# frank-xwang/InstanceDiffusion

Measured on AMD Instinct MI355X. Metric: images/sec at 512x512, 50 PLMS steps, N=8 instances (Multi-instance Sampler), higher is better.
Workload: dtype bf16; 1 GPU; C3: SD-1.5 InstanceDiffusion UNet (1.228B params, seeded random weights), 64x64 latent (512x512), 50 PLMS steps, CFG 7.5, N=8 boxes, MIS 0.36, alpha [0.8,0,0.2]; images_per_gpu=32, unet_forwards_per_image=406

## Files before the change

### include/idf.h

```cpp
#ifndef IDF_H_
#define IDF_H_

#include <stdint.h>

#ifdef __cplusplus
extern "C" {
#endif

#define IDF_ABI_VERSION 5

enum { IDF_BF16 = 0, IDF_F16 = 1 };
enum { IDF_E_ARG = -1, IDF_E_ALIGN = -2, IDF_E_UNSUPPORTED = -3 };

enum {
  IDF_EPI_BIAS     = 1,
  IDF_EPI_ROWBIAS  = 2,
  IDF_EPI_RES      = 4,
  IDF_EPI_GATE     = 8,
  IDF_EPI_SILU     = 16,
  IDF_EPI_GELU     = 32,
  IDF_EPI_GEGLU    = 64,
  IDF_EPI_OUT_F32  = 128,
  IDF_EPI_OUT_NCHW = 256,
  IDF_EPI_LN_ROW   = 512,
  IDF_EPI_LN_COL   = 1024,
  IDF_EPI_GEGLU_P32 = 2048
};

int idf_abi_version(void);
const char* idf_build_info(void);

enum { IDF_TUNE_GEMM_BIG = 0, IDF_TUNE_ATTN2 = 1, IDF_TUNE_GEMM_RING = 2, IDF_TUNE_BIG_MIN_EFF = 3, IDF_TUNE_ATTN8 = 4, IDF_TUNE_MLP = 5,
       IDF_TUNE_QKV_ROW = 6, IDF_TUNE_GEGLU_ROW = 7 };
int idf_set_tuning(int knob, int value);
enum { IDF_STAT_GEMM_BIG_LAUNCHES = 0, IDF_STAT_ATTN2_LAUNCHES = 1, IDF_STAT_GEMM_RING_LAUNCHES = 2, IDF_STAT_ATTN8_LAUNCHES = 3,
       IDF_STAT_GN_EPI_LAUNCHES = 4 ,
       IDF_STAT_QKV_ROW_LAUNCHES = 6 ,
       IDF_STAT_GEGLU_ROW_LAUNCHES = 7  };
long long idf_get_stat(int stat);

typedef struct {
  const void* A; const void* W; void* out;
  const float* bias; const void* rowbias; const void* res; const float* gate;
  int M, N, K;
  int lda, ldw, ldo, ldr, ld_rowbias;
  int rows_per_batch;
  int batch; long long strideA, strideW, strideO, strideR;
  int epi; int dtype;
  void* ws; long long ws_bytes;
  const float* ln_stats; long long stride_ln_stats;
  const float* ln_c;
  const float* ln_d;
  float* out_stats; float out_stats_eps;
  float ln_eps; float* ln_stats_out;
  void* vt_out; int ld_vt; int vt_col0;
} idf_gemm_args;
int idf_gemm(const idf_gemm_args* a, void* stream);

typedef struct {
  const void* x; int ldx;
  const float* ln_stats;
  const void* w1; int ldw1;
  const float* cd;
  const void* w2p; int ldw2;
  const float* b2;
  const float* gate;
  void* out; int ldo;
  int M, C;
  int dtype;
} idf_mlp_args;
int idf_mlp_geglu(const idf_mlp_args* a, void* stream);

int idf_row_stats(const void* x, int ldx, float* stats, int M, int C, float eps, int dtype, void* stream);

typedef struct {
  const void* x; const void* W; void* out;
  const float* bias; const void* rowbias; const void* res;
  int B, Hin, Win, Cin, Cout;
  int stride;
  int upsample;
  int ldx, ldo, ldr, ld_rowbias;
  int n_valid;
  int epi; int dtype;
  void* ws; long long ws_bytes;
  float* gn_partial;
} idf_conv3x3_args;
int idf_conv3x3(const idf_conv3x3_args* a, void* stream);
int idf_conv3x3_down(const idf_conv3x3_args* a, void* stream);
int idf_conv_up2x_folded(const idf_conv3x3_args* a, void* stream);

int idf_conv_in(const float* x_nchw, const float* w , const float* bias, void* out,
                int B, int Cin, int H, int W, int Cout, int dtype, void* stream);

typedef struct {
// ... 64 lines not shown
```

### instancediffusion_amd/_lib.py

```python
from __future__ import annotations

import ctypes as C
import os

_HERE = os.path.dirname(os.path.abspath(__file__))
LIB_PATH = os.environ.get("IDF_LIB_PATH", os.path.join(_HERE, "libidf_gfx950.so"))

IDF_BF16, IDF_F16 = 0, 1
IDF_STAT_GEMM_BIG_LAUNCHES, IDF_STAT_ATTN2_LAUNCHES, IDF_STAT_GEMM_RING_LAUNCHES, IDF_STAT_ATTN8_LAUNCHES, IDF_STAT_GN_EPI_LAUNCHES = 0, 1, 2, 3, 4
IDF_STAT_QKV_ROW_LAUNCHES, IDF_STAT_GEGLU_ROW_LAUNCHES = 6, 7
IDF_TUNE_GEMM_BIG, IDF_TUNE_ATTN2, IDF_TUNE_GEMM_RING, IDF_TUNE_BIG_MIN_EFF, IDF_TUNE_ATTN8, IDF_TUNE_MLP, IDF_TUNE_QKV_ROW, IDF_TUNE_GEGLU_ROW = 0, 1, 2, 3, 4, 5, 6, 7
EPI_LN_ROW, EPI_LN_COL, EPI_GEGLU_P32 = 512, 1024, 2048
EPI_BIAS, EPI_ROWBIAS, EPI_RES, EPI_GATE, EPI_SILU, EPI_GELU, EPI_GEGLU, EPI_OUT_F32, EPI_OUT_NCHW = \
    1, 2, 4, 8, 16, 32, 64, 128, 256

vp, ll, ci, cf = C.c_void_p, C.c_longlong, C.c_int, C.c_float


class GemmArgs(C.Structure):
    _fields_ = [("A", vp), ("W", vp), ("out", vp), ("bias", vp), ("rowbias", vp), ("res", vp), ("gate", vp),
                ("M", ci), ("N", ci), ("K", ci),
                ("lda", ci), ("ldw", ci), ("ldo", ci), ("ldr", ci), ("ld_rowbias", ci),
                ("rows_per_batch", ci),
                ("batch", ci), ("strideA", ll), ("strideW", ll), ("strideO", ll), ("strideR", ll),
                ("epi", ci), ("dtype", ci), ("ws", vp), ("ws_bytes", ll),
                ("ln_stats", vp), ("stride_ln_stats", ll), ("ln_c", vp), ("ln_d", vp),
                ("out_stats", vp), ("out_stats_eps", cf),
                ("ln_eps", cf), ("ln_stats_out", vp),
                ("vt_out", vp), ("ld_vt", ci), ("vt_col0", ci)]


E_UNSUPPORTED = -3


class ConvArgs(C.Structure):
    _fields_ = [("x", vp), ("W", vp), ("out", vp), ("bias", vp), ("rowbias", vp), ("res", vp),
                ("B", ci), ("Hin", ci), ("Win", ci), ("Cin", ci), ("Cout", ci),
                ("stride", ci), ("upsample", ci),
                ("ldx", ci), ("ldo", ci), ("ldr", ci), ("ld_rowbias", ci),
                ("n_valid", ci), ("epi", ci), ("dtype", ci), ("ws", vp), ("ws_bytes", ll), ("gn_partial", vp)]


class AttnArgs(C.Structure):
    _fields_ = [("q", vp), ("ldq", ci), ("strideQ", ll), ("nq", ci),
                ("k0", vp), ("ldk0", ci), ("strideK0", ll), ("vt0", vp), ("ldv0", ci), ("strideV0", ll), ("n0", ci),
                ("k1", vp), ("ldk1", ci), ("strideK1", ll), ("vt1", vp), ("ldv1", ci), ("strideV1", ll), ("n1", ci),
                ("out", vp), ("ldo", ci), ("strideO", ll),
                ("B", ci), ("H", ci), ("d", ci), ("scale", cf), ("dtype", ci),
                ("qbits", vp), ("strideQb", ll), ("kbits0", vp), ("strideKb0", ll), ("kbits1", vp), ("strideKb1", ll)]


class MlpArgs(C.Structure):
    _fields_ = [("x", vp), ("ldx", ci), ("ln_stats", vp), ("w1", vp), ("ldw1", ci), ("cd", vp), ("w2p", vp), ("ldw2", ci),
                ("b2", vp), ("gate", vp), ("out", vp), ("ldo", ci), ("M", ci), ("C", ci), ("dtype", ci)]


SYMBOLS = {
    "idf_abi_version": (ci, []),
    "idf_build_info": (C.c_char_p, []),
    "idf_set_tuning": (ci, [ci, ci]),
    "idf_get_stat": (ll, [ci]),
    "idf_gemm": (ci, [C.POINTER(GemmArgs), vp]),
    "idf_conv3x3": (ci, [C.POINTER(ConvArgs), vp]),
    "idf_conv3x3_down": (ci, [C.POINTER(ConvArgs), vp]),
    "idf_conv_up2x_folded": (ci, [C.POINTER(ConvArgs), vp]),
    "idf_mlp_geglu": (ci, [C.POINTER(MlpArgs), vp]),
    "idf_conv_in": (ci, [vp, vp, vp, vp, ci, ci, ci, ci, ci, ci, vp]),
    "idf_attention": (ci, [C.POINTER(AttnArgs), vp]),
    "idf_groupnorm_ws_floats": (ll, [ci, ci]),
    "idf_groupnorm": (ci, [vp, vp, vp, vp, vp, ci, ci, ci, cf, ci, ci, vp]),
    "idf_groupnorm_stats": (ci, [vp, vp, ci, ci, ci, ci, ci, vp]),
    "idf_groupnorm_apply": (ci, [vp, vp, vp, vp, vp, ci, ci, ci, ci, cf, ci, ci, vp]),
    "idf_layernorm": (ci, [vp, ci, vp, ci, vp, vp, ci, ci, cf, ci, vp]),
    "idf_row_stats": (ci, [vp, ci, vp, ci, ci, cf, ci, vp]),
    "idf_layernorm_patch2": (ci, [vp, vp, ci, vp, vp, ci, ci, ci, ci, cf, ci, vp]),
    "idf_seg_in_conv": (ci, [vp, vp, vp, vp, ci, ci, ci, ci, ci, vp]),
    "idf_dwconv7x7": (ci, [vp, vp, vp, vp, ci, ci, ci, ci, ci, vp]),
    "idf_scaleu_concat": (ci, [vp, vp, vp, vp, vp, vp, ci, ci, ci, ci, ci, ci, vp]),
    "idf_timestep_embedding": (ci, [vp, vp, ci, ci, ci, vp]),
    "idf_unifusion_embed": (ci, [vp, vp, vp, vp, vp, vp, vp, vp, ci, ci, ci, ci, vp]),
    "idf_cfg_combine": (ci, [vp, vp, cf, vp, ll, vp]),
    "idf_plms_update": (ci, [vp, vp, vp, vp, vp, vp, ci, cf, cf, cf, vp, ll, vp]),
    "idf_mis_merge": (ci, [vp, vp, vp, ci, ci, ci, ci, ci, ci, vp]),
    "idf_cast_f32_to_16": (ci, [vp, vp, ll, ci, vp]),
    "idf_softmax_rows": (ci, [vp, vp, ll, ci, ll, ll, cf, ci, vp]),
    "idf_pointwise_nchw": (ci, [vp, vp, vp, vp, ci, ci, ci, ll, cf, vp]),
    "idf_vae_posterior": (ci, [vp, vp, vp, vp, cf, vp, vp, ci, ci, ci, ll, vp]),
}

# ... 34 lines not shown
```

### instancediffusion_amd/csrc/gemm_conv.hip

```cpp
#include "gemm_core.h"
#include "attn_core.h"
#include <cstdlib>

using namespace idfcore;

namespace {

#ifndef IDF_GEMM_BIG_DEFAULT
#define IDF_GEMM_BIG_DEFAULT 1
#endif
constexpr int LSTR = 72;

template <int DT, int BM, int BN, int WM, int WN, int KLOOP_LDS_BYTES>
__device__ __forceinline__ void tile_epilogue(const CoreParams& p, f32x16 (&acc)[WN / 32][WM / 32], unsigned short* smem,
                                              int m0, int n0, int bz, int wm, int wn, int lane, int wave) {
  constexpr int TM = WM / 32, TN = WN / 32;
  const int l31 = lane & 31, hi = lane >> 5;
  constexpr int CSTR = WN + 4;
  static_assert(4 * WM * CSTR * 4 <= KLOOP_LDS_BYTES, "C staging must fit in the allocated LDS");
  __syncthreads();
  float* Cl = reinterpret_cast<float*>(smem) + wave * (WM * CSTR);
#pragma unroll
  for (int a = 0; a < TN; ++a)
#pragma unroll
// ... 812 lines not shown
    g_ring_tiles = value;
    return prev;
  }
  if (knob == IDF_TUNE_BIG_MIN_EFF) {
    if (value < 1 || value > 100) return IDF_E_ARG;
    return idf_big_min_eff_pct(value);
  }
  if (knob == IDF_TUNE_ATTN2) {
    if (value < 0 || value > 6) return IDF_E_ARG;
    return idf_attn2_set_mode(value);
  }
  if (knob == IDF_TUNE_ATTN8) {
    if (value < 0 || value > 6) return IDF_E_ARG;
    return idf_attn8_set_mode(value);
  }
  if (knob == IDF_TUNE_GEGLU_ROW) {
    if (value < 0 || value > 1) return IDF_E_ARG;
    return idf_gegluw_set_mode(value);
  }
  if (knob == IDF_TUNE_QKV_ROW) {
    if (value < 0 || value > 1) return IDF_E_ARG;
    return idf_qkvw_set_mode(value);
  }
  if (knob == IDF_TUNE_MLP) {
    if (value < 0 || value > 1) return IDF_E_ARG;
    return idf_mlp_set_mode(value);
  }
  return IDF_E_ARG;
}

extern "C" long long idf_get_stat(int stat) {
  if (stat == IDF_STAT_GEMM_BIG_LAUNCHES) return idf_stat_big_launches.load();
  if (stat == IDF_STAT_ATTN2_LAUNCHES) return idf_stat_attn2_launches.load();
  if (stat == IDF_STAT_GEMM_RING_LAUNCHES) return idf_stat_ring_launches.load();
  if (stat == IDF_STAT_ATTN8_LAUNCHES) return idf_stat_attn8_launches.load();
  if (stat == IDF_STAT_GN_EPI_LAUNCHES) return idf_stat_gn_epi_launches.load();
  if (stat == IDF_STAT_QKV_ROW_LAUNCHES) return idf_stat_qkvw_launches.load();
  if (stat == IDF_STAT_GEGLU_ROW_LAUNCHES) return idf_stat_gegluw_launches.load();
  return -1;
}

extern "C" int idf_gemm(const idf_gemm_args* a, void* stream) {
  if (!a || !a->A || !a->W || !a->out) return IDF_E_ARG;
  if (a->M <= 0 || a->N <= 0 || a->K <= 0 || (a->K % BK) != 0) return IDF_E_ARG;
  if ((a->lda % 8) || (a->ldw % 8) || !aligned16(a->A) || !aligned16(a->W)) return IDF_E_ALIGN;
  if ((a->epi & IDF_EPI_GATE) && !(a->epi & IDF_EPI_RES)) return IDF_E_ARG;
// ... 153 lines not shown
```

### instancediffusion_amd/csrc/gemm_core.h

```cpp
#pragma once
#include "common.h"
#include <atomic>

namespace idfcore {

struct CoreParams {
  const unsigned short* W; int ldw; long long strideW; int N;
  const unsigned short* A; int lda; long long strideA; int M; int K;
  int Hin, Win, Cin, Ho, Wo, stride, up;
  void* out; int ldo; long long strideO;
  const float* bias; const unsigned short* rowbias; int ld_rowbias; int rows_per_batch;
  const unsigned short* res; int ldr; long long strideR;
  const float* gate; int epi; int n_valid;
  float* ws; size_t ws_bytes; int splitk; int kt_per_slice;
  int full_items; int kt_full; int tail_m0; int tail_rows;
  const float* ln_stats; long long stride_ln_stats; const float* ln_c; const float* ln_d;
  float ln_eps; float* ln_stats_out;
  unsigned short* vt_out; int ld_vt; int vt_col0;
  float* stat_parts; int parts;
  float* gn_partial; int gn_hw;
  int tile_walk; int dephase; int dephase_units; int epi_vmcnt;
  int pad_lo;
  int fold_tiles;
};
// ... 79 lines not shown
    if (full && ((p.ldo & 7) == 0)) {
      *reinterpret_cast<u32x4*>(o) = pack8<DT>(v);
    } else {
#pragma unroll
      for (int e = 0; e < 8; ++e) if (n + e < p.N) o[e] = Elem<DT>::from_f32(v[e]);
    }
  }
}


}

#define IDF_BIG_UNSUPPORTED (-100)
extern std::atomic<long long> idf_stat_big_launches;
int idf_launch_big(const idfcore::CoreParams& p, int dtype, bool conv, bool force, hipStream_t s, int* splitk_out,
                   int* parts_out = nullptr, int* tail_m0_out = nullptr, int* gst_out = nullptr);
int idf_launch_big_fold(const idfcore::CoreParams& p, int dtype, bool force, hipStream_t s);
int idf_launch_qkv320w(const idfcore::CoreParams& p, int dtype, hipStream_t s);
int idf_launch_geglu640w(const idfcore::CoreParams& p, int dtype, hipStream_t s);
int idf_gegluw_set_mode(int v);
int idf_launch_qkv640w(const idfcore::CoreParams& p, int dtype, hipStream_t s);
int idf_qkvw_set_mode(int v);
int idf_mlp_set_mode(int v);
int idf_big_min_eff_pct(int set);
int idf_num_cu();
int idf_stats_finalize(const float* stat_parts, int parts, int cols_per_part, float* out_stats, int M, float eps, hipStream_t s);
```

### instancediffusion_amd/engine.py

```python
from __future__ import annotations

import os
from typing import Dict, List, Optional, Sequence, Tuple

import torch

from .host.attention import SpatialTransformer
from .host.unet import Downsample, ResBlock, UNetModel, Upsample

LN_SELF_MODE = int(os.environ.get("IDF_LN_SELF", "1"))
if LN_SELF_MODE not in (0, 1, 2):
    raise ValueError(f"IDF_LN_SELF={LN_SELF_MODE}: must be 0, 1 or 2")
QKV_ROW = os.environ.get("IDF_QKV_ROW", "1") != "0"
OBJ_TOKENS = 184
MASK_RES = 64


def _round_up(x: int, m: int) -> int:
    return (x + m - 1) // m * m


GEGLU_PERIOD = int(os.environ.get("IDF_GEGLU_PERIOD", "32"))
if GEGLU_PERIOD not in (32, 64):
    raise ValueError(f"IDF_GEGLU_PERIOD={GEGLU_PERIOD}: must be 32 or 64")
MLP_FUSED = os.environ.get("IDF_MLP_FUSED", "1")
if MLP_FUSED not in ("0", "1"):
    raise ValueError(f"IDF_MLP_FUSED={MLP_FUSED}: must be 0 or 1")
MLP_FUSED = MLP_FUSED == "1" and GEGLU_PERIOD == 32
MLP_MIN_M = int(os.environ.get("IDF_MLP_MIN_M", "32768"))
PAIR_HOIST = os.environ.get("IDF_PAIR_HOIST", "1")
if PAIR_HOIST not in ("0", "1"):
    raise ValueError(f"IDF_PAIR_HOIST={PAIR_HOIST}: must be 0 or 1")
PAIR_HOIST = PAIR_HOIST == "1"
GN_EPI = os.environ.get("IDF_GN_EPI", "1")
if GN_EPI not in ("0", "1"):
    raise ValueError(f"IDF_GN_EPI={GN_EPI}: must be 0 or 1")
GN_EPI = GN_EPI == "1"
UP_FOLD = os.environ.get("IDF_UP_FOLD", "1")
if UP_FOLD not in ("0", "1"):
    raise ValueError(f"IDF_UP_FOLD={UP_FOLD}: must be 0 or 1")
UP_FOLD = UP_FOLD == "1"
DEBUG_PAIRED = os.environ.get("IDF_DEBUG_PAIRED", "0") == "1"


def pack_geglu(w: torch.Tensor, b: torch.Tensor, period: int = 64) -> Tuple[torch.Tensor, torch.Tensor]:
    n2, k = w.shape
    n = n2 // 2
    h = period // 2
    assert n % h == 0
    wv, wg = w[:n].reshape(n // h, h, k), w[n:].reshape(n // h, h, k)
    bv, bg = b[:n].reshape(n // h, h), b[n:].reshape(n // h, h)
    return torch.cat([wv, wg], dim=1).reshape(n2, k).contiguous(), torch.cat([bv, bg], dim=1).reshape(n2).contiguous()


def pack_conv3x3(w: torch.Tensor) -> torch.Tensor:
    co, ci = w.shape[0], w.shape[1]
    return w.permute(0, 2, 3, 1).reshape(co, 9 * ci).contiguous()


def pack_conv_up2x(w: torch.Tensor) -> torch.Tensor:
    assert w.dim() == 4 and tuple(w.shape[2:]) == (3, 3) and w.dtype == torch.float32
    co, ci = w.shape[0], w.shape[1]
    rows = ((w[:, :, 0], w[:, :, 1] + w[:, :, 2]), (w[:, :, 0] + w[:, :, 1], w[:, :, 2]))
    out = w.new_empty(4, co, 4 * ci)
    for py in range(2):
        for px in range(2):
            taps = []
            for ty in range(2):
                r = rows[py][ty]
                cols = (r[:, :, 0], r[:, :, 1] + r[:, :, 2]) if px == 0 else (r[:, :, 0] + r[:, :, 1], r[:, :, 2])
                taps += [cols[0], cols[1]]
            out[py * 2 + px] = torch.stack(taps, dim=1).reshape(co, 4 * ci)
    return out


class _Lin:
    __slots__ = ("w", "b")

    def __init__(self, w, b):
        self.w, self.b = w, b


class Cond:

    _next_uid = 0

    def __init__(self, B: int):
        Cond._next_uid += 1
        self.uid = Cond._next_uid
        self.B = B
        self.objs: Optional[torch.Tensor] = None
        self.k_ctx: List[torch.Tensor] = []
        self.vt_ctx: List[torch.Tensor] = []
        self.k_obj: List[torch.Tensor] = []
        self.vt_obj: List[torch.Tensor] = []
        self.n_ctx = 0
# ... 99 lines not shown
    def _pack_ff(self, ff, norm):
        w = ff.net[0].proj.weight.detach().float()
        g, b = norm.weight.detach().float(), norm.bias.detach().float()
        wp, dp = pack_geglu(w * g[None, :], ff.net[0].proj.bias.detach().float() + w @ b, GEGLU_PERIOD)
        w16 = self._w16(wp)
        f = dict(w1=w16, b1=self._f32(dp), c1=w16.float().sum(1).contiguous(), l2=self._lin(ff.net[2]))
        C = w.shape[1]
        if MLP_FUSED and hasattr(self.ops, "mlp_geglu") and self.ops.mlp_supported(128, C):
            f["cd"], f["w2p"] = self.ops.mlp_pack(w16, f["c1"], f["b1"], f["l2"].w)
        return f

    def _attn(self, a, norm, self_attn: bool):
        d = dict(out=self._lin(a.to_out[0]))
        if self_attn:
            w3, c3, d3 = self._fold_ln(torch.cat([a.to_q.weight.detach(), a.to_k.weight.detach(), a.to_v.weight.detach()], 0),
                                       None, norm)
            C2 = 2 * a.to_q.weight.shape[0]
            d["wqkv"], d["cqkv"], d["dqkv"] = w3, c3, d3
            d["wqk"], d["cqk"], d["dqk"] = w3[:C2], c3[:C2], d3[:C2]
            d["wv"], d["cv"], d["dv"] = w3[C2:], c3[C2:], d3[C2:]
        else:
            d["wq"], d["cq"], d["dq"] = self._fold_ln(a.to_q.weight, None, norm)
            d["wk"], d["wv"] = self._w16(a.to_k.weight), self._w16(a.to_v.weight)
        return d

    def _attn_kv_plain(self, a):
        return dict(wk=self._w16(a.to_k.weight), wv=self._w16(a.to_v.weight))

    def _pack_res(self, rb: ResBlock, emb_w: list, emb_b: list, off: list):
        p = dict(kind="res", cin=rb.channels, cout=rb.out_channels,
                 gn1=(self._f32(rb.in_layers[0].weight), self._f32(rb.in_layers[0].bias)),
                 conv1=self._conv(rb.in_layers[2]),
                 gn2=(self._f32(rb.out_layers[0].weight), self._f32(rb.out_layers[0].bias)),
                 conv2=self._conv(rb.out_layers[3]),
                 skip=None if isinstance(rb.skip_connection, torch.nn.Identity) else self._lin(rb.skip_connection),
                 emb_off=off[0])
        emb_w.append(rb.emb_layers[1].weight.detach().float())
        emb_b.append(rb.emb_layers[1].bias.detach().float())
        off[0] += rb.out_channels
        return p

    def _pack_st(self, st: SpatialTransformer, tanh_alphas: list):
        blk = st.transformer_blocks[0]
        fz = blk.fuser
        idx = len(tanh_alphas)
        tanh_alphas.append(torch.stack([torch.tanh(fz.alpha_attn.detach().float()),
# ... 347 lines not shown
        y = ops.gemm(g.view(M, C), p["proj_in"].w, self.buf("st.x", (M, C)), bias=p["proj_in"].b, out_stats=pqkv)
        att = self._self_attn(p["attn1"], y, st, B, N, C)
        ops.gemm(att.view(M, C), p["attn1"]["out"].w, y, bias=p["attn1"]["out"].b, res=y,
                 out_stats=pqkv if fuser_on else pre)
        if dup:
            x, y = self._dup(x, "st.x_in2"), self._dup(y.view(B, N, C), "st.x2").view(2 * M, C)
            if (pqkv if fuser_on else pre) is not None:
                st = self._dup(st.view(B, N, 2), "st.stats2").view(2 * M, 2)
                pre = st if pre is not None else None
                pqkv = st if pqkv is not None else None
                ffs = st if ffs is not None else None
            else:
                st = self.buf("st.stats", (2 * M, 2), torch.float32)
                ffs = st if ffs is not None else None
            B, M = 2 * B, 2 * M
        i = p["idx"]
        if fuser_on:
            vis = cond.vis if (cond.vis and N == MASK_RES * MASK_RES) else None
            att = self._self_attn(p["f_attn"], y, st, B, N, C, kv_extra=(cond.k_obj[i], cond.vt_obj[i]), vis=vis)
            ops.gemm(att.view(M, C), p["f_attn"]["out"].w, y, bias=p["f_attn"]["out"].b, res=y, gate=self.gates[i, 0:1],
                     out_stats=ffs)
            self._ff(p["f_ff"], y, st, M, C, gate=self.gates[i, 1:2], out_stats=pre)
        a2 = p["attn2"]
        q = ops.gemm(y, a2["wq"], self.buf("st.q", (M, C)), bias=a2["dq"],
                     ln_row=(None if own else st, a2["cq"])).view(B, N, C)
        att = self.buf("st.att", (B, N, C))
        ops.attention(q, cond.k_ctx[i], cond.vt_ctx[i], cond.n_ctx, att, self.heads)
        ops.gemm(att.view(M, C), a2["out"].w, y, bias=a2["out"].b, res=y, out_stats=ffs)
        self._ff(p["ff"], y, st, M, C)
        ops.gemm(y, p["proj_out"].w, x.view(M, C), bias=p["proj_out"].b, res=x.view(M, C))
        return x

    def _run_block(self, layers, h, x_nchw, emb_all, cond, fuser_on, out_role, dup_st: bool = False, gnp=None, next_kind=None):
        for j, p in enumerate(layers):
            k = p["kind"]
            nxt = layers[j + 1]["kind"] if j + 1 < len(layers) else next_kind
            norm_next = nxt in ("res", "st")
            if k == "conv_in":
                B, _, H, W = x_nchw.shape
                h = self.ops.conv_in(x_nchw, p["w"], p["b"], self.buf(out_role, (B, H, W, p["w"].shape[0])))
                gnp = None
            elif k == "res":
                h, gnp = self._res(p, h, emb_all, out_role, gnp, want_out=norm_next)
            elif k == "st":
                h = self._st(p, h, cond, fuser_on, dup=dup_st, gnp=gnp)
                gnp = None
            elif k == "down":
                B, H, W, C = h.shape
                Ho, Wo = (H + 1) // 2, (W + 1) // 2
                gnp = self._gnp("gnp.out", B, Ho * Wo, C) if norm_next else None
                h = self.ops.conv3x3(h, p["conv"].w, self.buf(out_role, (B, Ho, Wo, C)), bias=p["conv"].b, stride=2, gn_partial=gnp)
# ... 132 lines not shown
```

### instancediffusion_amd/ops.py

```python
from __future__ import annotations

import ctypes as C
from typing import Optional

import torch

from . import _lib
from ._lib import (EPI_BIAS, EPI_GATE, EPI_GEGLU, EPI_GEGLU_P32, EPI_GELU, EPI_LN_COL, EPI_LN_ROW, EPI_OUT_F32, EPI_OUT_NCHW,
                   EPI_RES, EPI_ROWBIAS, EPI_SILU)

_DT = {torch.bfloat16: _lib.IDF_BF16, torch.float16: _lib.IDF_F16}


def _p(t: Optional[torch.Tensor]):
    return None if t is None else C.c_void_p(t.data_ptr())


def _rows2d(t: torch.Tensor):
    assert t.stride(-1) == 1 or t.shape[-1] == 1, "last dim must be contiguous"
    return t.stride(-2), (t.stride(0) if t.dim() == 3 else 0)


class HipOps:

# ... 115 lines not shown

    @classmethod
    def mlp_pack(cls, w1p16, c1, d1, w2_16):
        n2 = c1.numel()
        cd = torch.cat([c1.float().view(n2 // 64, 64), d1.float().view(n2 // 64, 64)], dim=1).contiguous()
        perm = torch.tensor(cls.MLP_W2_PERM, device=w2_16.device)
        n, k = w2_16.shape
        w2p = w2_16.view(n, k // 16, 16).index_select(2, perm).reshape(n, k).contiguous()
        return cd, w2p

    def mlp_geglu(self, x, stats, w1, cd, w2p, b2, out, *, gate=None):
        M, Cc = x.shape
        assert self.mlp_supported(M, Cc) and out.shape == x.shape and x.stride(-1) == 1 and out.stride(-1) == 1
        assert stats.is_contiguous() and stats.dtype == torch.float32 and stats.numel() == 2 * M
        assert w1.shape == (8 * Cc, Cc) and w2p.shape == (Cc, 4 * Cc) and cd.is_contiguous() and cd.numel() == 16 * Cc
        assert w1.stride(-1) == 1 and w2p.stride(-1) == 1 and b2.dtype == torch.float32 and cd.dtype == torch.float32
        args = _lib.MlpArgs(x=x.data_ptr(), ldx=x.stride(0), ln_stats=stats.data_ptr(), w1=w1.data_ptr(), ldw1=w1.stride(0),
                            cd=cd.data_ptr(), w2p=w2p.data_ptr(), ldw2=w2p.stride(0), b2=b2.data_ptr(),
                            gate=None if gate is None else gate.data_ptr(), out=out.data_ptr(), ldo=out.stride(0), M=M, C=Cc,
                            dtype=self.dt)
        _lib.check(self.lib.idf_mlp_geglu(C.byref(args), self._stream()), "idf_mlp_geglu")
        return out

    @staticmethod
    def gn_partial_shape(B, HW, C):
        return (B, HW // 64, 32, 2) if (HW % 64 == 0 and C % 32 == 0) else None

    def conv3x3(self, x, w, out, *, bias=None, rowbias=None, res=None, stride=1, upsample=0, n_valid=0, gn_partial=None):
        B, H, W_, Cin = x.shape
        assert x.stride(-1) == 1 and x.stride(1) == W_ * x.stride(2) and x.stride(0) == H * x.stride(1)
        Cout = w.shape[0]
        epi = 0
        if bias is not None:
            epi |= EPI_BIAS
        if rowbias is not None:
            epi |= EPI_ROWBIAS
        if res is not None:
            epi |= EPI_RES
        if n_valid:
            epi |= EPI_OUT_NCHW
            assert out.dtype == torch.float32 and out.is_contiguous()
            ldo = 0
        else:
            ldo = out.stride(2)
        args = _lib.ConvArgs(
            x=x.data_ptr(), W=w.data_ptr(), out=out.data_ptr(),
# ... 222 lines not shown
```

Before: 2.157 img/s.

## Fuse cross-attention block (LN-folded Q proj, attention, out proj) into one kernel

Adds a persistent fused kernel for the C=320, 8-head cross-attention sub-block. It computes row LayerNorm stats, the folded-LN Q projection, softmax attention over the small text context, the output projection with bias and residual, and the next LN stats, all in one pass. This replaces two GEMMs plus an attention launch and the Q and attention intermediates written to and read back from HBM. The cost is a complex custom kernel with AGPR-resident accumulators and weights packed into a special layout. It only applies to the 320-channel levels, and the fallback path is kept.

```diff
diff --git a/include/idf.h b/include/idf.h
--- a/include/idf.h
+++ b/include/idf.h
@@ -31,7 +31,7 @@
 const char* idf_build_info(void);
 
 enum { IDF_TUNE_GEMM_BIG = 0, IDF_TUNE_ATTN2 = 1, IDF_TUNE_GEMM_RING = 2, IDF_TUNE_BIG_MIN_EFF = 3, IDF_TUNE_ATTN8 = 4, IDF_TUNE_MLP = 5,
-       IDF_TUNE_QKV_ROW = 6, IDF_TUNE_GEGLU_ROW = 7 };
+       IDF_TUNE_QKV_ROW = 6, IDF_TUNE_GEGLU_ROW = 7, IDF_TUNE_XATTN_ROW = 9  };
 int idf_set_tuning(int knob, int value);
 enum { IDF_STAT_GEMM_BIG_LAUNCHES = 0, IDF_STAT_ATTN2_LAUNCHES = 1, IDF_STAT_GEMM_RING_LAUNCHES = 2, IDF_STAT_ATTN8_LAUNCHES = 3,
        IDF_STAT_GN_EPI_LAUNCHES = 4 ,
@@ -70,6 +70,21 @@
   int dtype;
 } idf_mlp_args;
 int idf_mlp_geglu(const idf_mlp_args* a, void* stream);
+
+typedef struct {
+  const void* x; int ldx;
+  const void* wq; const void* wo;
+  const float* cq; const float* dq; const float* bo;
+  const void* k; int ldk; long long strideK;
+  const void* vt; int ldv; long long strideV;
+  int n_ctx; int rows_per_batch;
+  float scale; float ln_eps;
+  void* out; int ldo;
+  float* out_stats; float out_stats_eps;
+  int M, C, heads;
+  int dtype;
+} idf_xattn_args;
+int idf_xattn_block(const idf_xattn_args* a, void* stream);
 
 int idf_row_stats(const void* x, int ldx, float* stats, int M, int C, float eps, int dtype, void* stream);
 
diff --git a/instancediffusion_amd/_lib.py b/instancediffusion_amd/_lib.py
--- a/instancediffusion_amd/_lib.py
+++ b/instancediffusion_amd/_lib.py
@@ -10,6 +10,7 @@
 IDF_STAT_GEMM_BIG_LAUNCHES, IDF_STAT_ATTN2_LAUNCHES, IDF_STAT_GEMM_RING_LAUNCHES, IDF_STAT_ATTN8_LAUNCHES, IDF_STAT_GN_EPI_LAUNCHES = 0, 1, 2, 3, 4
 IDF_STAT_QKV_ROW_LAUNCHES, IDF_STAT_GEGLU_ROW_LAUNCHES = 6, 7
 IDF_TUNE_GEMM_BIG, IDF_TUNE_ATTN2, IDF_TUNE_GEMM_RING, IDF_TUNE_BIG_MIN_EFF, IDF_TUNE_ATTN8, IDF_TUNE_MLP, IDF_TUNE_QKV_ROW, IDF_TUNE_GEGLU_ROW = 0, 1, 2, 3, 4, 5, 6, 7
+IDF_TUNE_XATTN_ROW = 9
 EPI_LN_ROW, EPI_LN_COL, EPI_GEGLU_P32 = 512, 1024, 2048
 EPI_BIAS, EPI_ROWBIAS, EPI_RES, EPI_GATE, EPI_SILU, EPI_GELU, EPI_GEGLU, EPI_OUT_F32, EPI_OUT_NCHW = \
     1, 2, 4, 8, 16, 32, 64, 128, 256
@@ -55,6 +56,14 @@
                 ("b2", vp), ("gate", vp), ("out", vp), ("ldo", ci), ("M", ci), ("C", ci), ("dtype", ci)]
 
 
+class XattnArgs(C.Structure):
+    _fields_ = [("x", vp), ("ldx", ci), ("wq", vp), ("wo", vp), ("cq", vp), ("dq", vp), ("bo", vp),
+                ("k", vp), ("ldk", ci), ("strideK", ll), ("vt", vp), ("ldv", ci), ("strideV", ll),
+                ("n_ctx", ci), ("rows_per_batch", ci), ("scale", cf), ("ln_eps", cf),
+                ("out", vp), ("ldo", ci), ("out_stats", vp), ("out_stats_eps", cf),
+                ("M", ci), ("C", ci), ("heads", ci), ("dtype", ci)]
+
+
 SYMBOLS = {
     "idf_abi_version": (ci, []),
     "idf_build_info": (C.c_char_p, []),
@@ -65,6 +74,7 @@
     "idf_conv3x3_down": (ci, [C.POINTER(ConvArgs), vp]),
     "idf_conv_up2x_folded": (ci, [C.POINTER(ConvArgs), vp]),
     "idf_mlp_geglu": (ci, [C.POINTER(MlpArgs), vp]),
+    "idf_xattn_block": (ci, [C.POINTER(XattnArgs), vp]),
     "idf_conv_in": (ci, [vp, vp, vp, vp, ci, ci, ci, ci, ci, ci, vp]),
     "idf_attention": (ci, [C.POINTER(AttnArgs), vp]),
     "idf_groupnorm_ws_floats": (ll, [ci, ci]),
diff --git a/instancediffusion_amd/csrc/gemm_conv.hip b/instancediffusion_amd/csrc/gemm_conv.hip
--- a/instancediffusion_amd/csrc/gemm_conv.hip
+++ b/instancediffusion_amd/csrc/gemm_conv.hip
@@ -858,6 +858,10 @@
     if (value < 0 || value > 1) return IDF_E_ARG;
     return idf_qkvw_set_mode(value);
   }
+  if (knob == IDF_TUNE_XATTN_ROW) {
+    if (value < 0 || value > 1) return IDF_E_ARG;
+    return idf_xattnw_set_mode(value);
+  }
   if (knob == IDF_TUNE_MLP) {
     if (value < 0 || value > 1) return IDF_E_ARG;
     return idf_mlp_set_mode(value);
diff --git a/instancediffusion_amd/csrc/gemm_core.h b/instancediffusion_amd/csrc/gemm_core.h
--- a/instancediffusion_amd/csrc/gemm_core.h
+++ b/instancediffusion_amd/csrc/gemm_core.h
@@ -125,6 +125,7 @@
 int idf_launch_qkv640w(const idfcore::CoreParams& p, int dtype, hipStream_t s);
 int idf_qkvw_set_mode(int v);
 int idf_mlp_set_mode(int v);
+int idf_xattnw_set_mode(int v);
 int idf_big_min_eff_pct(int set);
 int idf_num_cu();
 int idf_stats_finalize(const float* stat_parts, int parts, int cols_per_part, float* out_stats, int M, float eps, hipStream_t s);
diff --git a/instancediffusion_amd/csrc/xattn_fused.hip b/instancediffusion_amd/csrc/xattn_fused.hip
--- /dev/null
+++ b/instancediffusion_amd/csrc/xattn_fused.hip
@@ -0,0 +1,365 @@
+#include "mw_row.h"
+
+using namespace idfcore;
+using namespace idfmw;
+
+namespace {
+
+constexpr int XA_BM = 128, XA_C = 320, XA_H = 8, XA_D = 40, XA_DP = 48, XA_NK = 96;
+constexpr int XA_WQ_BYTES = 5 * XA_DP * 128;
+constexpr int XA_WO_BYTES = XA_C * XA_DP * 2;
+constexpr int XA_KSTR = 96, XA_VSTR = 208;
+constexpr int XA_WQ_OFF = 0, XA_WO_OFF = XA_WQ_OFF + XA_WQ_BYTES, XA_K_OFF = XA_WO_OFF + XA_WO_BYTES;
+constexpr int XA_V_OFF = XA_K_OFF + XA_NK * XA_KSTR, XA_CD_OFF = XA_V_OFF + XA_DP * XA_VSTR;
+constexpr int XA_B_OFF = XA_CD_OFF + 2 * XA_H * XA_DP * 4, XA_STG_OFF = (XA_B_OFF + XA_C * 4 + 127) & ~127;
+constexpr int XA_SMEM = XA_STG_OFF + 4 * 2 * 2048;
+constexpr int XA_PIECES = XA_WQ_BYTES / 1024;
+static_assert(XA_WQ_BYTES == XA_WO_BYTES && XA_WQ_BYTES % 1024 == 0, "one piece loop serves both images");
+constexpr int XA_AHEAD = 3;
+constexpr int XA_NAGPR = 240;
+
+struct XaParams {
+  const unsigned short* x; int ldx;
+  const char* wq; const char* wo;
+  const float* cq; const float* dq; const float* bo;
+  const unsigned short* k; int ldk; long long sK;
+  const unsigned short* vt; int ldv; long long sV;
+  int n_ctx, rows_per_batch;
+  float scale_log2, ln_eps, out_eps;
+  unsigned short* out; int ldo;
+  float* stats;
+  int M;
+};
+
+template <int DT> __device__ __forceinline__ float xa_lo(unsigned v) { return Elem<DT>::to_f32((unsigned short)(v & 0xffffu)); }
+template <int DT> __device__ __forceinline__ float xa_hi(unsigned v) { return Elem<DT>::to_f32((unsigned short)(v >> 16)); }
+
+template <int DT>
+__global__ __launch_bounds__(256, 1) void xattn320w_kernel(const XaParams p, const int tiles) {
+  asm volatile("" ::: "a0", "a239");
+  extern __shared__ __attribute__((aligned(128))) char smem[];
+  const RowLane rl = mw_row_lane();
+  const int tid = rl.tid, lane = rl.lane, wave = rl.wave, l31 = rl.l31, hi = rl.hi;
+  const int G = gridDim.x;
+  const unsigned smem_lds = lds_u32(smem);
+
+  int tile = mw_first_tile(G);
+  if (tile >= tiles) return;
+
+  const unsigned lane16 = (unsigned)lane * 16u;
+  auto dma = [&](const char* src, unsigned dst) {
+    for (int pc = wave; pc < XA_PIECES; pc += 4) mw_dma_rt(src + pc * 1024, lane16, dst + (unsigned)(pc * 1024));
+  };
+  int k_src[2], k_dst[2], v_src[2], v_dst[2], v_valid[2];
+#pragma unroll
+  for (int i = 0; i < 2; ++i) {
+    const int id = tid + 256 * i;
+    const int kr = id / 5, kc = id - 5 * kr;
+    const bool kok = kr < XA_NK;
+    k_src[i] = kok ? (kr < p.n_ctx ? kr : p.n_ctx - 1) * p.ldk + 8 * kc : -1;
+    k_dst[i] = XA_K_OFF + kr * XA_KSTR + 16 * kc;
+    const int vr = id / 12, vc = id - 12 * vr;
+    v_src[i] = vr < XA_D ? vr * p.ldv + 8 * vc : -1;
+    v_dst[i] = XA_V_OFF + vr * XA_VSTR + (vc >> 1) * 32 + (vc & 1) * 8;
+    v_valid[i] = p.n_ctx - 8 * vc;
+  }
+
+  for (int i = tid; i < XA_H * XA_DP; i += 256) {
+    reinterpret_cast<float*>(smem + XA_CD_OFF)[i] = p.cq[i];
+    reinterpret_cast<float*>(smem + XA_CD_OFF)[XA_H * XA_DP + i] = p.dq[i];
+  }
+  for (int i = tid; i < XA_C; i += 256) reinterpret_cast<float*>(smem + XA_B_OFF)[i] = p.bo[i];
+  for (int i = tid; i < (XA_CD_OFF - XA_K_OFF) / 16; i += 256) reinterpret_cast<u32x4*>(smem + XA_K_OFF)[i] = u32x4{0u, 0u, 0u, 0u};
+  __syncthreads();
+  for (int i = tid; i < XA_VSTR / 2; i += 256) reinterpret_cast<unsigned short*>(smem + XA_V_OFF + XA_D * XA_VSTR)[i] = Elem<DT>::from_f32(1.0f);
+  dma(p.wq, smem_lds + (unsigned)XA_WQ_OFF);
+  auto row_ptr = [&](int t) { return p.x + (size_t)(t * XA_BM + wave * 32 + l31) * p.ldx + 8 * hi; };
+  {
+    const unsigned short* xr = row_ptr(tile);
+    mw_static_for<20>([&](auto kc) { mw_load_x<decltype(kc)::value>(xr); });
+  }
+
+  const float sc = p.scale_log2;
+  const int wq_r1 = 32 + (l31 & 15);
+  const char* const wq0 = smem + XA_WQ_OFF + l31 * 128;
+  const char* const wq1 = smem + XA_WQ_OFF + wq_r1 * 128;
+  const int sw0 = (l31 >> 1) & 7, sw1 = (wq_r1 >> 1) & 7;
+  const char* const kf = smem + XA_K_OFF + l31 * XA_KSTR + 16 * hi;
+  const char* const vf0 = smem + XA_V_OFF + l31 * XA_VSTR + 16 * hi;
+  const char* const vf1 = smem + XA_V_OFF + wq_r1 * XA_VSTR + 16 * hi;
+  const char* const wof = smem + XA_WO_OFF + l31 * (XA_DP * 2) + 16 * hi;
+  const float* const cdt = reinterpret_cast<const float*>(smem + XA_CD_OFF) + 4 * hi;
+
+  for (;;) {
+    asm volatile("s_waitcnt vmcnt(0)" ::: "memory");
+    __builtin_amdgcn_s_barrier();
+    asm volatile("" ::: "memory");
+    float mu, rstd;
+    {
+      const float piv = __shfl(xa_lo<DT>(mw_agpr_read<MW_XA>()), l31, 64);
+      float s1 = 0.0f, s2 = 0.0f;
+      mw_static_for<80>([&](auto rc) {
+        const unsigned v = mw_agpr_read<MW_XA + decltype(rc)::value>();
+        const float a = xa_lo<DT>(v) - piv, b = xa_hi<DT>(v) - piv;
+        s1 += a + b;
+        s2 = fmaf(a, a, fmaf(b, b, s2));
+      });
+      s1 += __shfl_xor(s1, 32, 64);
+      s2 += __shfl_xor(s2, 32, 64);
+      const float m1 = s1 * (1.0f / XA_C);
+      mu = piv + m1;
+      rstd = rsqrtf(fmaxf(fmaf(-m1, m1, s2 * (1.0f / XA_C)), 0.0f) + p.ln_eps);
+    }
+    const float nmu = -mu;
+    mw_static_for<160>([&](auto rc) { mw_agpr_write<MW_OA + decltype(rc)::value>(0u); });
+
+    const int b = (tile * XA_BM) / p.rows_per_batch;
+    const unsigned short* const kb = p.k + (size_t)b * p.sK;
+    const unsigned short* const vb = p.vt + (size_t)b * p.sV;
+
+    for (int h = 0; h < XA_H; ++h) {
+      dma(p.wo + (size_t)h * XA_WO_BYTES, smem_lds + (unsigned)XA_WO_OFF);
+      u32x4 kreg[2], vreg[2];
+#pragma unroll
+      for (int i = 0; i < 2; ++i) {
+        kreg[i] = vreg[i] = u32x4{0u, 0u, 0u, 0u};
+        if (k_src[i] >= 0) kreg[i] = *reinterpret_cast<const u32x4*>(kb + h * XA_D + k_src[i]);
+        if (v_src[i] >= 0) vreg[i] = *reinterpret_cast<const u32x4*>(vb + (size_t)(h * XA_D) * p.ldv + v_src[i]);
+      }
+      f32x16 qa0, qa1;
+      {
+        auto rd = [&](auto kc, const char* row, int sw) {
+          constexpr int ks = decltype(kc)::value, kt = ks >> 2, sl = 2 * (ks & 3);
+          return *reinterpret_cast<const u32x4*>(row + kt * (XA_DP * 128) + (((sl + hi) ^ sw) << 4));
+        };
+        u32x4 w0[XA_AHEAD], w1[XA_AHEAD];
+        mw_static_for<XA_AHEAD>([&](auto kc) { w0[decltype(kc)::value] = rd(kc, wq0, sw0); w1[decltype(kc)::value] = rd(kc, wq1, sw1); });
+        mw_static_for<20>([&](auto kc) {
+          constexpr int ks = decltype(kc)::value, sl = ks % XA_AHEAD;
+          mw_mf1<DT, ks, ks == 0>(qa0, w0[sl]);
+          mw_mf1<DT, ks, ks == 0>(qa1, w1[sl]);
+          if constexpr (ks + XA_AHEAD < 20) {
+            w0[sl] = rd(std::integral_constant<int, ks + XA_AHEAD>{}, wq0, sw0);
+            w1[sl] = rd(std::integral_constant<int, ks + XA_AHEAD>{}, wq1, sw1);
+          }
+        });
+      }
+      asm volatile("s_nop 15\n\ts_nop 15" : "+v"(qa0), "+v"(qa1));
+      u32x4 qf[3];
+      {
+        const float* const ch = cdt + h * XA_DP;
+        auto fold8 = [&](const f32x16& a, int r0, int row0) {
+          float v[8];
+#pragma unroll
+          for (int g = 0; g < 2; ++g) {
+            const f32x4 c4 = *reinterpret_cast<const f32x4*>(ch + row0 + 8 * g);
+            const f32x4 d4 = *reinterpret_cast<const f32x4*>(ch + XA_H * XA_DP + row0 + 8 * g);
+#pragma unroll
+            for (int e = 0; e < 4; ++e) v[4 * g + e] = fmaf(rstd, fmaf(nmu, c4[e], a[r0 + 4 * g + e]), d4[e]);
+          }
+          return pack8<DT>(v);
+        };
+        qf[0] = fold8(qa0, 0, 0);
+        qf[1] = fold8(qa0, 8, 16);
+        qf[2] = fold8(qa1, 0, 32);
+      }
+#pragma unroll
+      for (int i = 0; i < 2; ++i) {
+        if (k_src[i] >= 0) *reinterpret_cast<u32x4*>(smem + k_dst[i]) = kreg[i];
+        if (v_src[i] >= 0) {
+#pragma unroll
+          for (int w = 0; w < 4; ++w)
+            vreg[i][w] &= (v_valid[i] >= 2 * w + 2) ? 0xffffffffu : ((v_valid[i] == 2 * w + 1) ? 0x0000ffffu : 0u);
+          *reinterpret_cast<u32x2*>(smem + v_dst[i]) = u32x2{vreg[i][0], vreg[i][1]};
+          *reinterpret_cast<u32x2*>(smem + v_dst[i] + 16) = u32x2{vreg[i][2], vreg[i][3]};
+        }
+      }
+      asm volatile("s_waitcnt vmcnt(0) lgkmcnt(0)" ::: "memory");
+      __builtin_amdgcn_s_barrier();
+      asm volatile("" ::: "memory");
+
+      dma(p.wq + (size_t)((h + 1) & (XA_H - 1)) * XA_WQ_BYTES, smem_lds + (unsigned)XA_WQ_OFF);
+      f32x16 s[3];
+      const f32x16 zero = {0.f, 0.f, 0.f, 0.f, 0.f, 0.f, 0.f, 0.f, 0.f, 0.f, 0.f, 0.f, 0.f, 0.f, 0.f, 0.f};
+#pragma unroll
+      for (int kt = 0; kt < 3; ++kt) {
+        s[kt] = zero;
+#pragma unroll
+        for (int ks = 0; ks < 3; ++ks)
+          s[kt] = Elem<DT>::mfma32(*reinterpret_cast<const u32x4*>(kf + kt * 32 * XA_KSTR + ks * 32), qf[ks], s[kt]);
+      }
+      float mx = -INFINITY;
+#pragma unroll
+      for (int kt = 0; kt < 3; ++kt)
+#pragma unroll
+        for (int r = 0; r < 16; ++r) {
+          const int key = 32 * kt + 8 * (r >> 2) + 4 * hi + (r & 3);
+          s[kt][r] = key < p.n_ctx ? s[kt][r] : -INFINITY;
+          mx = fmaxf(mx, s[kt][r]);
+        }
+      mx = fmaxf(mx, __shfl_xor(mx, 32, 64));
+      const float m = mx * sc;
+#pragma unroll
+      for (int kt = 0; kt < 3; ++kt)
+#pragma unroll
+        for (int r = 0; r < 16; ++r) s[kt][r] = __builtin_amdgcn_exp2f(fmaf(s[kt][r], sc, -m));
+      f32x16 o0 = zero, o1 = zero;
+#pragma unroll
+      for (int kt = 0; kt < 3; ++kt)
+#pragma unroll
+        for (int k2 = 0; k2 < 2; ++k2) {
+          u32x4 pf;
+#pragma unroll
+          for (int w = 0; w < 4; ++w) pf[w] = pack2<DT>(s[kt][8 * k2 + 2 * w], s[kt][8 * k2 + 2 * w + 1]);
+          o0 = Elem<DT>::mfma32(*reinterpret_cast<const u32x4*>(vf0 + (2 * kt + k2) * 32), pf, o0);
+          o1 = Elem<DT>::mfma32(*reinterpret_cast<const u32x4*>(vf1 + (2 * kt + k2) * 32), pf, o1);
+        }
+      const float inv = 1.0f / __shfl(o1[4], l31, 64);
+      u32x4 of[3];
+      {
+        float v[8];
+#pragma unroll
+        for (int r = 0; r < 8; ++r) v[r] = o0[r] * inv;
+        of[0] = pack8<DT>(v);
+#pragma unroll
+        for (int r = 0; r < 8; ++r) v[r] = o0[8 + r] * inv;
+        of[1] = pack8<DT>(v);
+#pragma unroll
+        for (int r = 0; r < 8; ++r) v[r] = o1[r] * inv;
+        of[2] = pack8<DT>(v);
+      }
+      {
+        auto rd = [&](auto ic) {
+          constexpr int i = decltype(ic)::value;
+          return *reinterpret_cast<const u32x4*>(wof + (i % 10) * 32 * (XA_DP * 2) + (i / 10) * 32);
+        };
+        u32x4 wf[2 * XA_AHEAD];
+        mw_static_for<2 * XA_AHEAD>([&](auto ic) { wf[decltype(ic)::value] = rd(ic); });
+        mw_static_for<30>([&](auto ic) {
+          constexpr int i = decltype(ic)::value, sl = i % (2 * XA_AHEAD);
+          mw_mf2<DT, i % 10>(wf[sl], of[i / 10]);
+          if constexpr (i + 2 * XA_AHEAD < 30) wf[sl] = rd(std::integral_constant<int, i + 2 * XA_AHEAD>{});
+        });
+      }
+      asm volatile("s_waitcnt vmcnt(0)" ::: "memory");
+      __builtin_amdgcn_s_barrier();
+      asm volatile("" ::: "memory");
+    }
+    asm volatile("s_nop 15\n\ts_nop 15\n\ts_nop 7" ::: "memory");
+
+    const int next = tile + G;
+    const bool has_next = next < tiles;
+    const unsigned short* const xn = row_ptr(has_next ? next : tile);
+    char* const stg = smem + XA_STG_OFF + wave * 4096;
+    const int sl_row = lane >> 2, sl_pc = lane & 3;
+    auto stg_f = [](int row) { return ((((row >> 2) ^ (row >> 3)) & 1) << 1) | (((row >> 1) ^ (row >> 3) ^ (row >> 4)) & 1); };
+    auto stg_at = [&](int slot, int row, int pc) { return reinterpret_cast<u32x4*>(stg + slot * 2048 + row * 64 + ((pc ^ stg_f(row)) << 4)); };
+    unsigned short* const orow = p.out + (size_t)(tile * XA_BM + wave * 32 + sl_row) * p.ldo + sl_pc * 8;
+    u32x4 po0, po1;
+    const char* const bl = smem + XA_B_OFF + 64 * hi;
+    float t1p[10], t2p[10];
+    mw_static_for<10>([&](auto ac) {
+      constexpr int a = decltype(ac)::value;
+      float acc[16];
+      mw_static_for<16>([&](auto rc) { acc[decltype(rc)::value] = __uint_as_float(mw_agpr_read<MW_OA + 16 * a + decltype(rc)::value>()); });
+      float v[16];
+#pragma unroll
+      for (int e = 0; e < 4; ++e) {
+        const auto s02 = __builtin_amdgcn_permlane32_swap(__float_as_uint(acc[e]), __float_as_uint(acc[8 + e]), false, false);
+        const auto s13 = __builtin_amdgcn_permlane32_swap(__float_as_uint(acc[4 + e]), __float_as_uint(acc[12 + e]), false, false);
+        v[e] = __uint_as_float(s02[0]); v[4 + e] = __uint_as_float(s02[1]);
+        v[8 + e] = __uint_as_float(s13[0]); v[12 + e] = __uint_as_float(s13[1]);
+      }
+#pragma unroll
+      for (int jq = 0; jq < 4; ++jq) {
+        const f32x4 bq = *reinterpret_cast<const f32x4*>(bl + (32 * a + 4 * jq) * 4);
+#pragma unroll
+        for (int e = 0; e < 4; ++e) v[4 * jq + e] += bq[e];
+      }
+      u32x4 r0, r1;
+      mw_static_for<4>([&](auto dc) {
+        constexpr int d = decltype(dc)::value;
+        const unsigned xa = mw_agpr_read<MW_XA + 4 * (2 * a) + d>(), xb = mw_agpr_read<MW_XA + 4 * (2 * a + 1) + d>();
+        const auto sw = __builtin_amdgcn_permlane32_swap(xa, xb, false, false);
+        r0[d] = sw[0]; r1[d] = sw[1];
+      });
+      if (has_next) { mw_load_x<2 * a>(xn); mw_load_x<2 * a + 1>(xn); }
+      float r[16];
+      unpack8<DT>(r0, r);
+      unpack8<DT>(r1, r + 8);
+#pragma unroll
+      for (int jq = 0; jq < 16; ++jq) v[jq] += r[jq];
+      const u32x4 pk0 = pack8<DT>(v), pk1 = pack8<DT>(v + 8);
+      unpack8<DT>(pk0, r);
+      unpack8<DT>(pk1, r + 8);
+      {
+        float d1[16], d2[16];
+#pragma unroll
+        for (int jq = 0; jq < 16; ++jq) { d1[jq] = r[jq] - mu; d2[jq] = d1[jq] * d1[jq]; }
+#pragma unroll
+        for (int w = 8; w >= 1; w >>= 1)
+#pragma unroll
+          for (int jq = 0; jq < w; ++jq) { d1[jq] += d1[jq + w]; d2[jq] += d2[jq + w]; }
+        t1p[a] = d1[0]; t2p[a] = d2[0];
+      }
+      if constexpr (a > 0) {
+        *reinterpret_cast<u32x4*>(orow + 32 * (a - 1)) = po0;
+        *reinterpret_cast<u32x4*>(orow + (size_t)16 * p.ldo + 32 * (a - 1)) = po1;
+      }
+      *stg_at(a & 1, l31, 2 * hi) = pk0;
+      *stg_at(a & 1, l31, 2 * hi + 1) = pk1;
+      asm volatile("" ::: "memory");
+      po0 = *stg_at(a & 1, sl_row, sl_pc); po1 = *stg_at(a & 1, sl_row + 16, sl_pc);
+      if constexpr (a == 9) {
+        *reinterpret_cast<u32x4*>(orow + 32 * a) = po0;
+        *reinterpret_cast<u32x4*>(orow + (size_t)16 * p.ldo + 32 * a) = po1;
+      }
+    });
+    if (p.stats) {
+      float t1 = ((t1p[0] + t1p[1]) + (t1p[2] + t1p[3])) + ((t1p[4] + t1p[5]) + (t1p[6] + t1p[7])) + (t1p[8] + t1p[9]);
+      float t2 = ((t2p[0] + t2p[1]) + (t2p[2] + t2p[3])) + ((t2p[4] + t2p[5]) + (t2p[6] + t2p[7])) + (t2p[8] + t2p[9]);
+      t1 += __shfl_xor(t1, 32, 64);
+      t2 += __shfl_xor(t2, 32, 64);
+      const float m1 = t1 * (1.0f / XA_C);
+      const float rs = rsqrtf(fmaxf(fmaf(-m1, m1, t2 * (1.0f / XA_C)), 0.0f) + p.out_eps);
+      if (hi == 0) reinterpret_cast<f32x2*>(p.stats)[(size_t)tile * XA_BM + wave * 32 + l31] = f32x2{mu + m1, rs};
+    }
+    if (!has_next) break;
+    tile = next;
+  }
+}
+
+MwKnob g_xattn_knob{"IDF_XATTN_ROW", 1};
+
+}
+
+int idf_xattnw_set_mode(int v) { return g_xattn_knob.set(v); }
+
+extern "C" int idf_xattn_block(const idf_xattn_args* a, void* stream) {
+  if (!a) return IDF_E_ARG;
+  if (!a->x || !a->wq || !a->wo || !a->cq || !a->dq || !a->bo || !a->k || !a->vt || !a->out) return IDF_E_ARG;
+  if (a->M <= 0 || a->C <= 0 || a->heads <= 0 || a->n_ctx <= 0 || a->rows_per_batch <= 0 || !(a->scale > 0.0f)) return IDF_E_ARG;
+  if (a->dtype != IDF_BF16 && a->dtype != IDF_F16) return IDF_E_ARG;
+  if (a->M % a->rows_per_batch) return IDF_E_ARG;
+  if (g_xattn_knob.get() == 0) return IDF_E_UNSUPPORTED;
+  if (a->C != XA_C || a->heads != XA_H || a->n_ctx > XA_NK) return IDF_E_UNSUPPORTED;
+  if ((a->M % XA_BM) || (a->rows_per_batch % XA_BM) || a->M < XA_BM * 2 * idf_num_cu()) return IDF_E_UNSUPPORTED;
+  if (a->ldx < XA_C || a->ldo < XA_C || a->ldk < XA_C || a->ldv < XA_NK) return IDF_E_ARG;
+  if ((a->ldx % 8) || (a->ldo % 8) || (a->ldk % 8) || (a->ldv % 8) || (a->strideK % 8) || (a->strideV % 8)) return IDF_E_ALIGN;
+  if (!aligned16(a->x) || !aligned16(a->out) || !aligned16(a->wq) || !aligned16(a->wo) || !aligned16(a->k) || !aligned16(a->vt) ||
+      !aligned16(a->cq) || !aligned16(a->dq) || !aligned16(a->bo) || (((uintptr_t)a->out_stats) & 7u))
+    return IDF_E_ALIGN;
+  if ((long long)XA_NK * a->ldk * 2 >= (1ll << 31) || (long long)XA_C * a->ldv * 2 >= (1ll << 31)) return IDF_E_UNSUPPORTED;
+  XaParams p;
+  p.x = static_cast<const unsigned short*>(a->x); p.ldx = a->ldx;
+  p.wq = static_cast<const char*>(a->wq); p.wo = static_cast<const char*>(a->wo);
+  p.cq = a->cq; p.dq = a->dq; p.bo = a->bo;
+  p.k = static_cast<const unsigned short*>(a->k); p.ldk = a->ldk; p.sK = a->strideK;
+  p.vt = static_cast<const unsigned short*>(a->vt); p.ldv = a->ldv; p.sV = a->strideV;
+  p.n_ctx = a->n_ctx; p.rows_per_batch = a->rows_per_batch;
+  p.scale_log2 = a->scale * 1.4426950408889634f; p.ln_eps = a->ln_eps; p.out_eps = a->out_stats_eps;
+  p.out = static_cast<unsigned short*>(a->out); p.ldo = a->ldo; p.stats = a->out_stats; p.M = a->M;
+  hipStream_t s = static_cast<hipStream_t>(stream);
+  return a->dtype == IDF_BF16 ? mw_row_launch<XaParams, xattn320w_kernel<IDF_BF16>, XA_SMEM, XA_BM>(p, s)
+                              : mw_row_launch<XaParams, xattn320w_kernel<IDF_F16>, XA_SMEM, XA_BM>(p, s);
+}
diff --git a/instancediffusion_amd/engine.py b/instancediffusion_amd/engine.py
--- a/instancediffusion_amd/engine.py
+++ b/instancediffusion_amd/engine.py
@@ -40,6 +40,7 @@
 if UP_FOLD not in ("0", "1"):
     raise ValueError(f"IDF_UP_FOLD={UP_FOLD}: must be 0 or 1")
 UP_FOLD = UP_FOLD == "1"
+XATTN_ROW = os.environ.get("IDF_XATTN_ROW", "1") != "0"
 DEBUG_PAIRED = os.environ.get("IDF_DEBUG_PAIRED", "0") == "1"
 
 
@@ -72,6 +73,59 @@
                 taps += [cols[0], cols[1]]
             out[py * 2 + px] = torch.stack(taps, dim=1).reshape(co, 4 * ci)
     return out
+
+
+XATTN_PERM = (0, 1, 2, 3, 8, 9, 10, 11, 4, 5, 6, 7, 12, 13, 14, 15)
+
+
+def xattn_rows(d: int) -> List[int]:
+    dp = _round_up(d, 16)
+    e = [16 * (r // 16) + XATTN_PERM[r % 16] for r in range(dp)]
+    return [x if x < d else -1 for x in e]
+
+
+def pack_xattn(wq: torch.Tensor, cq: torch.Tensor, dq: torch.Tensor, wo: torch.Tensor, bo: torch.Tensor, heads: int) -> Dict[str, torch.Tensor]:
+    C = wq.shape[0]
+    assert wq.shape == (C, C) and wo.shape == (C, C) and C % heads == 0 and C % 64 == 0
+    d = C // heads
+    rows = xattn_rows(d)
+    dp = len(rows)
+    dev = wq.device
+    idx = torch.tensor([max(r, 0) for r in rows], device=dev)
+    keep = torch.tensor([r >= 0 for r in rows], device=dev)
+    src = (torch.arange(heads, device=dev)[:, None] * d + idx[None, :]).reshape(-1)
+    wqp = (wq.index_select(0, src).view(heads, dp, C) * keep[None, :, None].to(wq.dtype))
+    cqp = cq.float().index_select(0, src).view(heads, dp) * keep[None, :]
+    dqp = dq.float().index_select(0, src).view(heads, dp) * keep[None, :]
+    wop = (wo.index_select(1, src).view(C, heads, dp) * keep[None, None, :].to(wo.dtype)).permute(1, 0, 2).contiguous()
+    t = wqp.view(heads, dp, C // 64, 8, 8).permute(0, 2, 1, 3, 4)
+    slot = torch.arange(8, device=dev)[None, :] ^ ((torch.arange(dp, device=dev)[:, None] >> 1) & 7)
+    img = t[:, :, torch.arange(dp, device=dev)[:, None], slot]
+    return dict(wq=img.reshape(heads, (C // 64) * dp * 64).contiguous(), cq=cqp.contiguous(), dq=dqp.contiguous(), wo=wop,
+                bo=bo.float().contiguous())
+
+
+def unpack_xattn(xa: Dict[str, torch.Tensor], C: int, heads: int):
+    d = C // heads
+    rows = xattn_rows(d)
+    dp = len(rows)
+    dev = xa["wq"].device
+    img = xa["wq"].view(heads, C // 64, dp, 8, 8)
+    slot = torch.arange(8, device=dev)[None, :] ^ ((torch.arange(dp, device=dev)[:, None] >> 1) & 7)
+    wqp = img[:, :, torch.arange(dp, device=dev)[:, None], slot].permute(0, 2, 1, 3, 4).reshape(heads, dp, C)
+    wq = xa["wq"].new_zeros(C, C)
+    wo = xa["wo"].new_zeros(C, C)
+    cq, dq = xa["cq"].new_zeros(C), xa["dq"].new_zeros(C)
+    pad = []
+    for r, e in enumerate(rows):
+        if e < 0:
+            pad += [wqp[:, r], xa["cq"][:, r], xa["dq"][:, r], xa["wo"][:, :, r]]
+            continue
+        ch = torch.arange(heads, device=dev) * d + e
+        wq[ch] = wqp[:, r]
+        cq[ch], dq[ch] = xa["cq"][:, r], xa["dq"][:, r]
+        wo[:, ch] = xa["wo"][:, :, r].t()
+    return wq, cq, dq, wo, pad
 
 
 class _Lin:
@@ -217,6 +271,9 @@
         else:
             d["wq"], d["cq"], d["dq"] = self._fold_ln(a.to_q.weight, None, norm)
             d["wk"], d["wv"] = self._w16(a.to_k.weight), self._w16(a.to_v.weight)
+            C = a.to_q.weight.shape[0]
+            if XATTN_ROW and hasattr(self.ops, "xattn_block") and C == 320 and self.heads == 8 and d["out"].b is not None:
+                d["xattn"] = pack_xattn(d["wq"], d["cq"], d["dq"], d["out"].w, d["out"].b, self.heads)
         return d
 
     def _attn_kv_plain(self, a):
@@ -610,11 +667,13 @@
                      out_stats=ffs)
             self._ff(p["f_ff"], y, st, M, C, gate=self.gates[i, 1:2], out_stats=pre)
         a2 = p["attn2"]
-        q = ops.gemm(y, a2["wq"], self.buf("st.q", (M, C)), bias=a2["dq"],
-                     ln_row=(None if own else st, a2["cq"])).view(B, N, C)
-        att = self.buf("st.att", (B, N, C))
-        ops.attention(q, cond.k_ctx[i], cond.vt_ctx[i], cond.n_ctx, att, self.heads)
-        ops.gemm(att.view(M, C), a2["out"].w, y, bias=a2["out"].b, res=y, out_stats=ffs)
+        if "xattn" not in a2 or not ops.xattn_block(y, a2["xattn"], cond.k_ctx[i], cond.vt_ctx[i], cond.n_ctx, N, self.heads, y,
+                                                    out_stats=ffs):
+            q = ops.gemm(y, a2["wq"], self.buf("st.q", (M, C)), bias=a2["dq"],
+                         ln_row=(None if own else st, a2["cq"])).view(B, N, C)
+            att = self.buf("st.att", (B, N, C))
+            ops.attention(q, cond.k_ctx[i], cond.vt_ctx[i], cond.n_ctx, att, self.heads)
+            ops.gemm(att.view(M, C), a2["out"].w, y, bias=a2["out"].b, res=y, out_stats=ffs)
         self._ff(p["ff"], y, st, M, C)
         ops.gemm(y, p["proj_out"].w, x.view(M, C), bias=p["proj_out"].b, res=x.view(M, C))
         return x
diff --git a/instancediffusion_amd/ops.py b/instancediffusion_amd/ops.py
--- a/instancediffusion_amd/ops.py
+++ b/instancediffusion_amd/ops.py
@@ -161,6 +161,32 @@
         _lib.check(self.lib.idf_mlp_geglu(C.byref(args), self._stream()), "idf_mlp_geglu")
         return out
 
+    def xattn_block(self, x, xa, k, vt, n_ctx, rows_per_batch, heads, out, *, out_stats=None, out_stats_eps=1e-5, ln_eps=1e-5) -> bool:
+        M, Cc = x.shape
+        assert out.shape == x.shape and x.stride(-1) == 1 and out.stride(-1) == 1 and x.dtype == self.dtype and out.dtype == self.dtype
+        assert k.dim() == 3 and vt.dim() == 3 and k.stride(-1) == 1 and vt.stride(-1) == 1 and k.dtype == self.dtype and vt.dtype == self.dtype
+        assert k.shape[0] == vt.shape[0] == M // rows_per_batch and k.shape[1] >= n_ctx and k.shape[2] == Cc and vt.shape[1] == Cc
+        d = Cc // heads
+        dp = (d + 15) // 16 * 16
+        for name, shape, dt in (("wq", (heads, 5 * dp * 64), self.dtype), ("wo", (heads, Cc, dp), self.dtype),
+                                ("cq", (heads, dp), torch.float32), ("dq", (heads, dp), torch.float32), ("bo", (Cc,), torch.float32)):
+            t = xa[name]
+            assert tuple(t.shape) == shape and t.dtype == dt and t.is_contiguous(), name
+        if out_stats is not None:
+            assert out_stats.is_contiguous() and out_stats.dtype == torch.float32 and out_stats.numel() == 2 * M
+        args = _lib.XattnArgs(
+            x=x.data_ptr(), ldx=x.stride(0), wq=xa["wq"].data_ptr(), wo=xa["wo"].data_ptr(), cq=xa["cq"].data_ptr(),
+            dq=xa["dq"].data_ptr(), bo=xa["bo"].data_ptr(), k=k.data_ptr(), ldk=k.stride(1), strideK=k.stride(0),
+            vt=vt.data_ptr(), ldv=vt.stride(1), strideV=vt.stride(0), n_ctx=n_ctx, rows_per_batch=rows_per_batch,
+            scale=float(d) ** -0.5, ln_eps=float(ln_eps), out=out.data_ptr(), ldo=out.stride(0),
+            out_stats=None if out_stats is None else out_stats.data_ptr(), out_stats_eps=float(out_stats_eps),
+            M=M, C=Cc, heads=heads, dtype=self.dt)
+        rc = self.lib.idf_xattn_block(C.byref(args), self._stream())
+        if rc == _lib.E_UNSUPPORTED:
+            return False
+        _lib.check(rc, "idf_xattn_block")
+        return True
+
     @staticmethod
     def gn_partial_shape(B, HW, C):
         return (B, HW // 64, 32, 2) if (HW % 64 == 0 and C % 32 == 0) else None
```

Measured after the change: 2.156 img/s. No clear change (-0.0%).
